# visionml/pytracking

Hardware: AMD Instinct MI355X
Metric: frames/sec DiMP-50 online track (288x288, 5 SD iters) (higher is better)
Workload: dtype f32; 1 GPU; BASELINE configs[1]: DiMP-50 single sequence per GPU; per frame classify(1x512x18x18) + arg-max + memory insert + DiMPSteepestDescentGN(5 it) over n=50x512x18x18, K=4; sequences_per_gpu=1, parallelism=1 independent sequences

## Files before the change

include/pt_hot.h:

```cpp
#ifndef PT_HOT_H
#define PT_HOT_H

#include <stddef.h>
#include <stdint.h>

#ifdef __cplusplus
extern "C" {
#endif

typedef enum pt_status {
    PT_OK = 0,
    PT_ERR_NULL = -1,
    PT_ERR_SHAPE = -2,
    PT_ERR_UNSUPPORTED = -3,
    PT_ERR_WORKSPACE = -4,
    PT_ERR_LAUNCH = -5
} pt_status;

const char* pt_strerror(int status);
int pt_abi_version(void);


size_t pt_apply_filter_ws_bytes(int n, int C, int H, int W, int KH, int KW, int OH, int OW);
int pt_apply_filter_f32(const float* feat, long feat_stride_n, const float* filt, float* scores,
                        int n, int C, int H, int W, int KH, int KW, int OH, int OW,
                        void* ws, size_t ws_bytes, void* stream);

size_t pt_feat_transpose_ws_bytes(int n, int C, int H, int W, int KH, int KW, int OH, int OW);
int pt_feat_transpose_f32(const float* feat, long feat_stride_n, const float* inp, float* grad,
                          int n, int C, int H, int W, int KH, int KW, int OH, int OW,
                          void* ws, size_t ws_bytes, void* stream);


enum { PT_SD_DIMP = 0, PT_SD_DIMP_L2 = 1, PT_SD_PRDIMP = 2 };
enum { PT_ACT_RELU = 0, PT_ACT_BENTPAR = 1 };
enum { PT_MASK_SIGMOID = 0, PT_MASK_LINEAR = 1 };

typedef struct pt_sd_params {
    int   kind;
    float step_length;
    float reg;
    float alpha_eps;
    float feat_stride;
    int   num_bins;
    float bin_displacement;
    const float* label_lut;
    const float* mask_lut;
    const float* spatial_lut;
    int   mask_act;
    int   score_act;
    float act_param;
    float gauss_sigma;
    float hinge_threshold;
    float uni_weight;
    int   normalize_label;
    float label_shrink;
    int   has_softmax_reg;
    float softmax_reg;
    float label_threshold;
} pt_sd_params;

size_t pt_sd_ws_bytes(int n, int C, int H, int W, int K);
int pt_sd_solve_f32(const pt_sd_params* p, const float* w_in, const float* feat, long feat_stride_n,
                    const float* bb, const float* sample_weight,
                    int n, int C, int H, int W, int K, int num_iter,
                    float* w_iters, float* losses, void* ws, size_t ws_bytes, void* stream);

int pt_sd_solve_batch_f32(const pt_sd_params* p, int S, const float* const* w_in, const float* const* feat, long feat_stride_n,
                          const float* const* bb, const float* const* sample_weight, int n, int C, int H, int W, int K,
                          int num_iter, float* const* w_iters, float* const* losses, void* const* ws, size_t ws_bytes_each,
                          void* stream, void* const* aux_streams, int n_aux);

typedef struct {
    int   score_act;
    float act_param;
// ... 226 lines not shown
```

pytracking_amd/_lib.py:

```python
import ctypes
import os
import subprocess

_HERE = os.path.dirname(os.path.abspath(__file__))
LIB_PATH = os.environ.get("PT_HOT_LIB", os.path.join(_HERE, "libpt_hot.so"))
SOURCES = ["filter_kernels.hip", "fast_passes.hip", "sd_solver.hip", "mf_kernels.hip", "lwl_solver.hip", "atom_cg.hip", "atom_gn.hip", "tomp.hip", "localize.hip", "iou_refine.hip", "prroi.hip", "patch.hip", "frame_full.hip", "api.hip", "gn_hinge.hip", "tcm.hip"]
HEADERS = ["common.h", "pt_internal.h", "rbuild.h", "sd_common.h", "mfma_gemm.h", "prroi_dev.h", "localize_dev.h", "frame_mid.h", os.path.join("..", "..", "include", "pt_hot.h")]
HIPCC_FLAGS = ["--offload-arch=gfx950", "-O3", "-std=c++17", "-fPIC", "-Wno-pass-failed", "-mllvm", "-amdgpu-kernarg-preload-count=14"]

PT_SD_DIMP, PT_SD_DIMP_L2, PT_SD_PRDIMP = 0, 1, 2
PT_ERR_NULL, PT_ERR_SHAPE, PT_ERR_UNSUPPORTED, PT_ERR_WORKSPACE, PT_ERR_LAUNCH = -1, -2, -3, -4, -5
PT_ACT_RELU, PT_ACT_BENTPAR = 0, 1
PT_MASK_SIGMOID, PT_MASK_LINEAR = 0, 1

class IouDims(ctypes.Structure):
    _fields_ = [(n, ctypes.c_int) for n in ("C3", "C4", "I3", "I4", "H3", "W3", "H4", "W4")]


class PatchGeom(ctypes.Structure):
    _fields_ = [(n, ctypes.c_int) for n in ("df", "os0", "os1", "tl0", "tl1", "crop_h", "crop_w")]


class AugDesc(ctypes.Structure):
    _fields_ = ([(n, ctypes.c_int) for n in ("kind", "pad_top", "pad_left", "th", "tw", "fs0", "fs1", "tap_off0", "tap_off1",
                                             "reserved")] + [("m", ctypes.c_double * 6)])


PT_AUG_IDENTITY, PT_AUG_FLIP_H, PT_AUG_FLIP_V, PT_AUG_BLUR, PT_AUG_SCALE, PT_AUG_ROTATE = range(6)
PT_AUG_MAX_TAPS = 256


class LocalizeParams(ctypes.Structure):
    _fields_ = ([(n, ctypes.c_double) for n in ("target_not_found_threshold", "uncertain_threshold", "hard_sample_threshold")]
                + [(n, ctypes.c_float) for n in ("distractor_threshold", "hard_negative_threshold", "target_not_found_f32",
                                                 "disp_threshold", "center_r", "center_c", "ratio_r", "ratio_c")]
                + [(n, ctypes.c_float * 8) for n in ("scale", "neigh_r", "neigh_c", "prev_r", "prev_c")])


class LocalizeState(ctypes.Structure):
    _fields_ = ([(n, ctypes.c_double) for n in ("target_not_found_threshold", "uncertain_threshold", "hard_sample_threshold",
                                                "distractor_threshold", "hard_negative_threshold",
                                                "target_neighborhood_scale", "dispalcement_scale")]
                + [(n, ctypes.c_float * 2) for n in ("kernel_size", "img_support_sz", "target_sz", "pos")]
                + [("sample_scales", ctypes.c_float * 8), ("sample_pos", ctypes.c_float * 16)])


PT_LOC_FLAGS = ("normal", "hard_negative", "uncertain", "not_found")


class FrameGlue(ctypes.Structure):
    _fields_ = [("image_sz", ctypes.c_float * 2), ("img_sample_sz", ctypes.c_float * 2), ("target_inside_ratio", ctypes.c_double),
                ("box_jitter_pos", ctypes.c_double), ("box_jitter_sz", ctypes.c_double), ("use_classifier", ctypes.c_int),
                ("num_random", ctypes.c_int), ("rand_u", ctypes.c_float * 60)]


PT_FRAME_HOST_FLOATS = 128


class TompDims(ctypes.Structure):
    _fields_ = [(n, ctypes.c_int) for n in ("d_model", "nhead", "dim_ff", "n_enc", "n_dec", "H", "W", "max_res")]


EXPORTS = [
    "pt_strerror", "pt_abi_version",
    "pt_apply_filter_ws_bytes", "pt_apply_filter_f32",
    "pt_feat_transpose_ws_bytes", "pt_feat_transpose_f32",
    "pt_sd_ws_bytes", "pt_sd_solve_f32",
    "pt_atom_cg_ws_bytes", "pt_atom_cg_f32", "pt_atom_gn_ws_bytes", "pt_atom_gn_f32",
    "pt_prroi_fwd_f32", "pt_prroi_bwd_feat_f32", "pt_prroi_bwd_coor_f32",
    "pt_track_frame_ws_bytes", "pt_track_frame_f32", "pt_track_frame_chain_f32", "pt_track_frame_flush_f32",
    "pt_apply_filter_mf_ws_bytes", "pt_apply_filter_mf_f32", "pt_feat_transpose_mf_ws_bytes", "pt_feat_transpose_mf_f32",
    "pt_lwl_ws_bytes", "pt_lwl_gn_solve_f32",
    "pt_tomp_param_floats", "pt_tomp_prepared_floats", "pt_tomp_prepare_f32", "pt_tomp_posenc_f32", "pt_tomp_predict_ws_bytes", "pt_tomp_predict_f32", "pt_tomp_linear_f32",
    "pt_tomp_bbreg_param_floats", "pt_tomp_bbreg_ws_bytes", "pt_tomp_bbreg_f32",
    "pt_clf_head_ws_bytes", "pt_clf_head_f32", "pt_max2d_f32", "pt_localize_f32", "pt_localize_decide_f32",
    "pt_localize_constants_f32", "pt_localize_advanced_f32", "pt_localize_advanced_sync_f32",
    "pt_iou_param_floats", "pt_iou_prepared_floats", "pt_iou_prepare_f32", "pt_iou_refine_ws_bytes", "pt_iou_refine_f32", "pt_iou_refine_sync_f32",
    "pt_track_frame_replay_pass_f32", "pt_sample_patch_f32", "pt_augment_patches_f32", "pt_track_frame_head_ws_bytes", "pt_track_frame_head_f32",
    "pt_track_frame_full_ws_bytes", "pt_track_frame_full_f32", "pt_track_frame_full_launch_f32", "pt_host_buffer_forget",
    "pt_track_frame_full_dyn_bytes", "pt_track_frame_full_dyn_fill_f32", "pt_host_wait_word_f32",
    "pt_sd_solve_batch_f32", "pt_stream_probe_f32",
    "pt_gn_hinge_ws_bytes", "pt_gn_hinge_solve_f32", "pt_gn_hinge_route",
    "pt_tcm_peaks_f32", "pt_tcm_desc_ws_bytes", "pt_tcm_desc_f32",
    "pt_tcm_match_weight_floats", "pt_tcm_match_ws_bytes", "pt_tcm_match_f32",
]

PT_TCM_MAX_POINTS, PT_TCM_MAX_LAYERS = 64, 32


class TcmMatchParams(ctypes.Structure):
    _fields_ = ([(n, ctypes.c_int) for n in ("M", "N", "n_layers")] + [("layer_types", ctypes.c_uint)]
                + [(n, ctypes.c_int) for n in ("skip_gnn", "sinkhorn_iters")] + [("filter_threshold", ctypes.c_float)]
                + [("kpt_center0", ctypes.c_float * 2), ("kpt_scale0", ctypes.c_float), ("kpt_center1", ctypes.c_float * 2),
                   ("kpt_scale1", ctypes.c_float), ("weight_floats", ctypes.c_size_t)])


class GnHingeParams(ctypes.Structure):
    _fields_ = [("score_act", ctypes.c_int)] + [(n, ctypes.c_float) for n in ("act_param", "hinge_threshold", "activation_leak",
                                                                             "filter_reg", "steplength_reg")]


class FramePending(ctypes.Structure):
    _fields_ = [("iters", ctypes.c_int), ("step_length", ctypes.c_float), ("reg_eps", ctypes.c_float)]


class SdParams(ctypes.Structure):
    _fields_ = [
        ("kind", ctypes.c_int), ("step_length", ctypes.c_float), ("reg", ctypes.c_float),
        ("alpha_eps", ctypes.c_float), ("feat_stride", ctypes.c_float),
        ("num_bins", ctypes.c_int), ("bin_displacement", ctypes.c_float),
        ("label_lut", ctypes.c_void_p), ("mask_lut", ctypes.c_void_p), ("spatial_lut", ctypes.c_void_p),
        ("mask_act", ctypes.c_int), ("score_act", ctypes.c_int), ("act_param", ctypes.c_float),
        ("gauss_sigma", ctypes.c_float), ("hinge_threshold", ctypes.c_float),
        ("uni_weight", ctypes.c_float), ("normalize_label", ctypes.c_int), ("label_shrink", ctypes.c_float),
        ("has_softmax_reg", ctypes.c_int), ("softmax_reg", ctypes.c_float), ("label_threshold", ctypes.c_float),
    ]


# ... 243 lines not shown
```

pytracking_amd/csrc/api.hip:

```cpp
#include <algorithm>
#include <atomic>
#include <chrono>
#include <mutex>
#include <utility>
#include <vector>
#include "common.h"
#include "pt_internal.h"

extern "C" const char* pt_strerror(int status) {
    switch (status) {
        case PT_OK: return "ok";
        case PT_ERR_NULL: return "required pointer is NULL";
        case PT_ERR_SHAPE: return "non-positive or inconsistent dimension";
        case PT_ERR_UNSUPPORTED: return "configuration not covered by the gfx950 kernels";
        case PT_ERR_WORKSPACE: return "workspace too small or not 256-byte aligned";
        case PT_ERR_LAUNCH: return "HIP launch failed";
        default: return "unknown status";
    }
}

extern "C" int pt_abi_version(void) { return 1; }

static std::atomic<const void*> g_pinned_seen[8];
static std::atomic<unsigned> g_pinned_next{0};
// ... 15 lines not shown
    for (auto& s : g_pinned_seen) {
        const void* cur = p;
        s.compare_exchange_strong(cur, nullptr, std::memory_order_acq_rel);
    }
}

bool pt_stream_events(void* main_stream, void* aux_stream, hipEvent_t* fork, hipEvent_t* join) {
    struct Key { int dev; void* main; void* aux; };
    struct Ent { Key k; hipEvent_t fork, join; };
    static std::mutex mu;
    static std::vector<Ent> pool;
    int dev = -1;
    if (hipGetDevice(&dev) != hipSuccess) { (void)hipGetLastError(); return false; }
    std::lock_guard<std::mutex> lk(mu);
    for (auto& e : pool)
        if (e.k.dev == dev && e.k.main == main_stream && e.k.aux == aux_stream) {
            if (fork) *fork = e.fork;
            if (join) *join = e.join;
            return true;
        }
    hipEvent_t a, b;
    if (hipEventCreateWithFlags(&a, hipEventDisableTiming) != hipSuccess) { (void)hipGetLastError(); return false; }
    if (hipEventCreateWithFlags(&b, hipEventDisableTiming) != hipSuccess) {
        (void)hipGetLastError();
        (void)hipEventDestroy(a);
        return false;
    }
    pool.push_back({{dev, main_stream, aux_stream}, a, b});
    if (fork) *fork = a;
    if (join) *join = b;
    return true;
}

int pt_poll_word(volatile float* word, float seq, const void* buf, void* stream) {
    const auto t0 = std::chrono::steady_clock::now();
    for (unsigned spin = 1;; ++spin) {
        if (*word == seq) break;
        __builtin_ia32_pause();
        if ((spin & 0xFFFF) == 0 && std::chrono::steady_clock::now() - t0 > std::chrono::seconds(2)) {
            pt_host_buffer_forget(buf);
            if (hipStreamSynchronize((hipStream_t)stream) != hipSuccess) return PT_ERR_LAUNCH;
            if (*word != seq) return PT_ERR_LAUNCH;
            break;
        }
    }
    __atomic_thread_fence(__ATOMIC_ACQUIRE);
    return PT_OK;
}

static int filt_check(int n, int C, int H, int W, int KH, int KW, int OH, int OW) {
    if (n <= 0 || C <= 0 || H <= 0 || W <= 0 || KH <= 0 || KW <= 0 || OH <= 0 || OW <= 0) return PT_ERR_SHAPE;
    if (OH > H + 2 * (KH / 2) - KH + 1 || OW > W + 2 * (KW / 2) - KW + 1) return PT_ERR_SHAPE;
    if (KH * KW > 16) return PT_ERR_UNSUPPORTED;
    return PT_OK;
}

extern "C" size_t pt_apply_filter_ws_bytes(int n, int C, int H, int W, int KH, int KW, int OH, int OW) {
    if (filt_check(n, C, H, W, KH, KW, OH, OW)) return 0;
    PtPlan p = pt_make_plan(n, C, H, W, KH, KW, OH, OW);
    size_t fl = pt_align_floats(pt_spart_floats(p));
    PtFast f = pt_fast_plan(n, C, H, W, KH, KW, OH, OW);
    if (f.ok) fl = std::max(fl, pt_align_floats(pt_fast_spart_floats(f)));
    return fl * sizeof(float);
}

extern "C" int pt_apply_filter_f32(const float* feat, long feat_stride_n, const float* filt, float* scores, int n, int C,
                                   int H, int W, int KH, int KW, int OH, int OW, void* ws, size_t ws_bytes,
                                   void* stream) {
    if (!feat || !filt || !scores || !ws) return PT_ERR_NULL;
    int rc = filt_check(n, C, H, W, KH, KW, OH, OW);
    if (rc) return rc;
    if (feat_stride_n < (long)C * H * W) return PT_ERR_SHAPE;
    if (ws_bytes < pt_apply_filter_ws_bytes(n, C, H, W, KH, KW, OH, OW) || ((uintptr_t)ws % 256) != 0)
        return PT_ERR_WORKSPACE;
    hipStream_t st = (hipStream_t)stream;
    float* spart = (float*)ws;
    PtFast f = pt_fast_plan(n, C, H, W, KH, KW, OH, OW);
    if (pt_fast_usable(f, feat, feat_stride_n, filt)) {
        rc = pt_launch_corr2(f, feat, feat_stride_n, filt, spart, st);
        if (rc) return rc;
        return pt_launch_sum_slices(spart, scores, f.KSC, (size_t)n * f.OO, st);
    }
    PtPlan p = pt_make_plan(n, C, H, W, KH, KW, OH, OW);
    rc = pt_launch_corr(p, feat, feat_stride_n, filt, spart, st);
    if (rc) return rc;
    return pt_launch_sum_slices(spart, scores, p.KS, (size_t)n * p.OO, st);
}

struct FtCarve { size_t R, gpart, total; };
static FtCarve ft_carve(const PtPlan& p) {
    FtCarve c;
    c.R = 0;
    c.gpart = pt_align_floats(pt_R_floats(p));
    c.total = c.gpart + pt_align_floats(pt_gpart_floats(p));
    return c;
}

extern "C" size_t pt_feat_transpose_ws_bytes(int n, int C, int H, int W, int KH, int KW, int OH, int OW) {
    if (filt_check(n, C, H, W, KH, KW, OH, OW)) return 0;
    PtPlan p = pt_make_plan(n, C, H, W, KH, KW, OH, OW);
    size_t fl = ft_carve(p).total;
    PtFast f = pt_fast_plan(n, C, H, W, KH, KW, OH, OW);
    if (f.ok) fl = std::max(fl, pt_align_floats(pt_fast_gpart_floats(f)));
    return fl * sizeof(float);
}

// ... 215 lines not shown
```

pytracking_amd/csrc/fast_passes.hip:

```cpp
#include "common.h"
#include "pt_internal.h"
#include "sd_common.h"

#ifndef PT_ADJ_WAVES
#define PT_ADJ_WAVES 8
#endif
#ifndef PT_ADJ_UMAX
#define PT_ADJ_UMAX (128 / PT_ADJ_WAVES)
#endif
#ifndef PT_ADJ_UMAX_WIDE
#define PT_ADJ_UMAX_WIDE (192 / PT_ADJ_WAVES)
#endif
#ifndef PT_C2_CD
#define PT_C2_CD 2
#endif
#ifndef PT_C2_MINW
#define PT_C2_MINW 6
#endif
#ifndef PT_ADJ_PD
#define PT_ADJ_PD 3
#endif

#ifdef PT_STAMPS
static unsigned long long* g_pt_stamps = nullptr;
extern "C" void pt_debug_set_stamps(void* p) { g_pt_stamps = (unsigned long long*)p; }
#define PT_STAMP_ARG unsigned long long* stamps;
#define PT_STAMP_SET(a) (a).stamps = g_pt_stamps
#define PT_STAMP(a, k)                                                                                       \
    do {                                                                                                     \
        if ((a).stamps && (threadIdx.x & 63) == 0)                                                           \
            (a).stamps[((long)blockIdx.x * 16 + (threadIdx.x >> 6)) * 8 + (k)] = (unsigned long long)wall_clock64(); \
    } while (0)
#else
#define PT_STAMP_ARG
#define PT_STAMP_SET(a)
#define PT_STAMP(a, k)
#endif
#if defined(PT_STAMPS) && PT_STAMPS == 2
#define PT_STAMP_A(a, k)
#define PT_STAMP_B(a, k) PT_STAMP(a, k)
#else
#define PT_STAMP_A(a, k) PT_STAMP(a, k)
#define PT_STAMP_B(a, k)
#endif

PtFast pt_fast_plan(int n, int C, int H, int W, int KH, int KW, int OH, int OW) {
    PtFast p;
    p.ok = 0;
    p.n = n; p.C = C; p.H = H; p.W = W; p.KH = KH; p.KW = KW; p.OH = OH; p.OW = OW;
    p.HW = H * W; p.KK = KH * KW; p.OO = OH * OW;
    if ((p.HW % 4) != 0 || W < 4 || p.KK > 16) return p;
    if (C != 64 && C != 128 && C != 256 && C != 512 && C != 1024) return p;
    if ((long)n * p.HW >= (1L << 20)) return p;
    if ((long)n * C * p.HW * 4 >= (1L << 31)) return p;
    p.Q = p.HW / 4;
    p.TF = p.Q / 16;
    p.rem = p.Q % 16;
    p.left = (p.rem > 0 && p.rem <= 4) ? 1 : 0;
    p.tiles = p.TF + ((p.rem > 0 && !p.left) ? 1 : 0);
    if (p.TF < 1 || p.tiles > 16) return p;
    p.nh = 2 * p.tiles <= 10 ? 2 : 1;
    p.CX = C / 8;
    p.KSC = 8;
    if (C == 64) { p.CX = C; p.KSC = 1; }
    p.spw = 1;
    if (p.nh == 2 && p.KSC == 8 && p.CX / 4 <= 16 && (n % 2) == 0 && 8 * n > 256) { p.nh = 1; p.spw = 2; }
    p.NK = p.CX / 4 / p.nh;
    if (p.NK > 16) return p;
    p.HWp = 64 * (p.TF + (p.rem > 0 ? 1 : 0)) + 4;
    p.corr_threads = p.spw * p.nh * p.tiles * 64;
    p.corr_lds = ((size_t)p.CX * 16 + (size_t)p.spw * p.nh * p.KK * p.HWp) * sizeof(float);
    p.sa_direct = (KH == 4 && KW == 4 && p.CX * 16 >= 2 * W + 2) ? 1 : 0;
    if (p.sa_direct && p.HWp < p.HW + 2 * W + 2) p.corr_lds += (size_t)(p.HW + 2 * W + 2 - p.HWp) * sizeof(float);
    if (p.corr_lds > 150 * 1024) return p;
    p.CB = C / 16;
    p.bpx = p.CB / 8;
    p.NG = (int)(((long)n * p.HW + 15) / 16);
    p.KSPL = 0;
    p.E = p.OO <= 384 ? 6 : (p.OO <= 576 ? 9 : 16);
    const int umax = p.E == 9 ? PT_ADJ_UMAX_WIDE : PT_ADJ_UMAX;
    for (int ks = 8; ks <= (p.CB < 8 ? 64 : 16); ks *= 2) {
        const int gper = pt_ceil_div(p.NG, ks), U = pt_ceil_div(gper, PT_ADJ_WAVES);
        if (U <= umax) { p.gper = gper; p.U = U; p.KSPL = pt_ceil_div(p.NG, gper); break; }
    }
    if (p.KSPL == 0) return p;
    p.PH = H + KH - 1;
    p.PW = W + KW - 1;
    while ((p.PW % 16) != 8) ++p.PW;
    p.ns_max = (p.gper * 16 + p.HW - 1) / p.HW + 1;
    p.zn = (KH - 1) * p.PW + KW + 4;
    while (((p.ns_max * p.PH * p.PW + p.zn) % 4) != 0) ++p.zn;
    p.adj_lds = ((size_t)p.ns_max * p.PH * p.PW + p.zn + (size_t)5 * 4 * PT_ADJ_WAVES * umax) * sizeof(float);
    if (p.adj_lds > 96 * 1024 || p.OO > 1024) return p;
    if (H > 255 || W > 255 || n > 65535 || p.gper > 65535 || p.PH > 63 || p.PW > 63 || p.zn > 255 || p.ns_max > 63 || KH > 7 || KW > 7)
        return p;
    p.ok = 1;
    return p;
}

__device__ __forceinline__ int fdiv(int v, float inv_d) { return (int)(((float)v + 0.5f) * inv_d); }

struct Corr2Args {
    pt_gcf feat; long stride_n; pt_gcf filt; pt_gf spart;
    int n, C, H, W, KH, KW, OH, OW, CX, TF, rem, tiles, HWp, nh, KSC;
    int sa_direct;
    pt_gcf gpart; int KSPL; pt_gcf w; float reg; float step; pt_gf g_out; pt_gf anum_part;
    int slot; pt_gcf src; pt_gf copy_dst;
    PT_STAMP_ARG
};

__device__ __forceinline__ float corr2_filter_elem(const Corr2Args& a, int KK, int cx0, int e, bool publish, float& gsq) {
    const int cl = e >> 4, tp = e & 15;
    const bool ok = tp < KK;
    const long ge = (long)(cx0 + cl) * KK + (ok ? tp : 0);
    float v;
    if (a.gpart) {
        const long CKK = (long)a.C * KK;
        v = 0.f;
        for (int k = 0; k < a.KSPL; ++k) v += a.gpart[(long)k * CKK + ge];
        v += a.reg * a.w[ge];
        if (ok) {
            gsq += v * v;
            if (publish) a.g_out[ge] = v;
        }
    } else {
        v = a.filt[ge];
    }
    return ok ? v : 0.f;
}

template <int NK, bool LEFT, int FUSE, bool K16, int NH>
__global__ __launch_bounds__(1024, (NK <= 8 && NH == 2 ? PT_C2_MINW : 4)) void k_corr2(const float* h_feat, long h_stride, const float* h_filt, const float* h_w, const float* h_src, int h_slot,
                                                                              unsigned h_dims, unsigned h_geo, unsigned h_aux, Corr2Args a_arg) {
    extern __shared__ __attribute__((aligned(16))) float lds[];
    __shared__ float scratch[16];
    PT_STAMP(a_arg, 0);
    constexpr int EPT = 2;
    constexpr int FP = FUSE > 0 ? FUSE : 1;
    const int hC = (int)(h_dims >> 16), HW = (int)(h_dims & 0xffffu);
    const int h_tiles = (int)(h_geo & 31u), h_TF = (int)((h_geo >> 5) & 31u), h_rem = (int)((h_geo >> 10) & 15u);
    const int h_KSPL = (int)((h_geo >> 14) & 63u);
    const bool ksc16 = ((h_geo >> 20) & 1u) != 0, ksc1 = ((h_geo >> 21) & 1u) != 0, pair = ((h_geo >> 22) & 1u) != 0;
    const int wps = NH * h_tiles;
    const int nthreads = (pair ? 2 : 1) * wps * 64;
    const int hCX = ksc1 ? hC : (ksc16 ? hC >> 4 : hC >> 3), hHWp = 64 * (h_TF + (h_rem > 0 ? 1 : 0)) + 4;
    const int b = blockIdx.x, xc = b & 7, q = b >> 3;
    const int x = ksc1 ? 0 : (ksc16 ? 2 * xc + (q & 1) : xc), i0 = ksc1 ? b : (ksc16 ? q >> 1 : q);
    const int KK = K16 ? 16 : a_arg.KH * a_arg.KW;
    const int lane = threadIdx.x & 63, wave = __builtin_amdgcn_readfirstlane(threadIdx.x >> 6);
    const int kq = lane >> 4, j = lane & 15;
    const int ws = (pair && wave >= wps) ? 1 : 0, wl = wave - ws * wps;
    const int i = pair ? 2 * i0 + ws : i0;
    const int h = wl >= h_tiles ? 1 : 0, t = wl - h * h_tiles;
    const int cx0 = hCX * x;
    const int nsl = hCX * 16;
    float* __restrict__ afilt = lds;
    float* __restrict__ Tl = lds + nsl + (long)(ws * NH + h) * KK * hHWp;
    const bool over = h_src != nullptr && i == h_slot;
    const float* __restrict__ fi = over ? h_src : h_feat + (long)i * h_stride;
    const bool publish = FUSE != 0 && i0 == 0;
    const int h_n = (int)(h_geo >> 23);
    float lz_q = 0.f, lz_an = 0.f;

    constexpr bool k16 = K16;
    const int n4 = nsl >> 1;
    const int e4 = min((int)threadIdx.x, n4 - 1);
    f32x2 part4[FP], wv4 = {0, 0};
    float part[EPT][FP], wv[EPT];
    long gev[EPT];
    bool okv[EPT];
    if (k16) {
        const long g4 = ((long)cx0 * 16 >> 1) + e4;
        if (FUSE > 0) {
            const unsigned ckk_b = (unsigned)hC * 16u * 4u;
            const __amdgpu_buffer_rsrc_t rg = pt_rsrc(h_filt, (unsigned)h_KSPL * ckk_b);
#pragma unroll
            for (int k = 0; k < FP; ++k)
                part4[k] = __builtin_bit_cast(f32x2, __builtin_amdgcn_raw_buffer_load_b64(rg, (unsigned)g4 * 8u, (unsigned)min(k, h_KSPL - 1) * ckk_b, 0));
            wv4 = ((const f32x2*)h_w)[g4];
        } else if (FUSE < 0) {
            part4[0] = ((const f32x2*)h_filt)[g4];
            wv4 = ((const f32x2*)h_w)[g4];
            const float* __restrict__ anp = h_w + h_aux;
            lz_an = lane < (ksc16 ? 16 : (ksc1 ? 1 : 8)) ? anp[lane] : 0.f;
            lz_q = lane < h_n ? anp[64 + lane] : 0.f;
        } else {
            part4[0] = ((const f32x2*)h_filt)[g4];
        }
    } else {
#pragma unroll
        for (int q = 0; q < EPT; ++q) {
            const int e = threadIdx.x + q * nthreads;
            const int ec = min(e, nsl - 1);
            const int cl = ec >> 4, tp = ec & 15;
            okv[q] = e < nsl && tp < KK;
            gev[q] = (long)(cx0 + cl) * KK + (tp < KK ? tp : 0);
            if (FUSE > 0) {
                const long CKK = (long)hC * KK;
#pragma unroll
                for (int k = 0; k < FP; ++k) part[q][k] = h_filt[(long)min(k, h_KSPL - 1) * CKK + gev[q]];
                wv[q] = h_w[gev[q]];
            } else {
                part[q][0] = h_filt[gev[q]];
            }
        }
    }

    constexpr int CD = NK < PT_C2_CD ? NK : PT_C2_CD;
    const int cbase = cx0 + 4 * (h * NK) + kq;
    const int pos = 64 * t + 4 * j;
    const bool pv = pos < HW;
    const __amdgpu_buffer_rsrc_t fr = pt_rsrc(fi, (unsigned)hC * HW * 4u);
    const unsigned fo = ((unsigned)cbase * HW + (pv ? pos : 0)) * 4u;
    const int lpos = 64 * h_TF + j;
    const bool lv = LEFT && t == 0 && j < 4 * h_rem;
    const unsigned lo = lv ? ((unsigned)cbase * HW + lpos) * 4u : 0xFFFFFFF0u - 64u * (unsigned)HW * 4u;
    f32x4 bq[NK];
    float bl[NK];
    auto ldq = [&](int k) {
        bq[k] = pt_bload4(fr, fo + (unsigned)(4 * k) * HW * 4u);
        if (LEFT && t == 0) bl[k] = pt_bload1(fr, lo + (unsigned)(4 * k) * HW * 4u);
    };
    if (LEFT && t == 0) {
#pragma unroll
        for (int k = 0; k < CD; ++k) bl[k] = pt_bload1(fr, lo + (unsigned)(4 * k) * HW * 4u);
    }
#pragma unroll
    for (int k = 0; k < CD; ++k) bq[k] = pt_bload4(fr, fo + (unsigned)(4 * k) * HW * 4u);
    __builtin_amdgcn_sched_barrier(0);
    const Corr2Args a = pt_late_args<Corr2Args>(56);
    PT_STAMP(a, 1);

    float gsq = 0.f;
    if (k16) {
        f32x2 v4;
        if (FUSE > 0) {
            v4 = (f32x2){0, 0};
#pragma unroll
            for (int k = 0; k < FP; ++k)
                if (k < h_KSPL) v4 += part4[k];
            v4 += a.reg * wv4;
            if ((int)threadIdx.x < n4) {
                gsq = v4[0] * v4[0] + v4[1] * v4[1];
                if (publish) ((f32x2*)a.g_out)[((long)cx0 * 16 >> 1) + e4] = v4;
            }
        } else if (FUSE < 0) {
            float qt = 0.f;
            for (int k = lane + 64; k < h_n; k += 64) qt += (h_w + h_aux)[64 + k];
            const float astep = sd_final_astep(lz_q, qt, lz_an, a.step, a.reg);
            v4 = (f32x2){sd_final_apply(part4[0][0], wv4[0], astep), sd_final_apply(part4[0][1], wv4[1], astep)};
            if ((int)threadIdx.x < n4 && publish) ((f32x2*)a.g_out)[((long)cx0 * 16 >> 1) + e4] = v4;
        } else {
            v4 = part4[0];
        }
        if ((int)threadIdx.x < n4) ((f32x2*)afilt)[e4] = v4;
        for (int q4 = threadIdx.x + nthreads; q4 < n4; q4 += nthreads)
            for (int m = 0; m < 2; ++m) afilt[2 * q4 + m] = corr2_filter_elem(a, KK, cx0, 2 * q4 + m, publish, gsq);
    } else {
#pragma unroll
        for (int q = 0; q < EPT; ++q) {
            const int e = threadIdx.x + q * nthreads;
            float v;
            if (FUSE > 0) {
                v = 0.f;
#pragma unroll
                for (int k = 0; k < FP; ++k) v += k < h_KSPL ? part[q][k] : 0.f;
                v += a.reg * wv[q];
                if (okv[q]) {
                    gsq += v * v;
                    if (publish) a.g_out[gev[q]] = v;
                }
            } else {
                v = part[q][0];
            }
            if (e < nsl) afilt[e] = okv[q] ? v : 0.f;
        }
        for (int e = threadIdx.x + EPT * nthreads; e < nsl; e += nthreads)
            afilt[e] = corr2_filter_elem(a, KK, cx0, e, publish, gsq);
    }
    if (FUSE > 0 && publish) {
        const float tot = block_sum(gsq, scratch, nthreads);
        if (threadIdx.x == 0) a.anum_part[x] = tot;
    }
    PT_STAMP(a, 2);
    __syncthreads();
    PT_STAMP(a, 3);

    f32x4 acc0 = {0, 0, 0, 0}, acc1 = {0, 0, 0, 0}, acc2 = {0, 0, 0, 0}, acc3 = {0, 0, 0, 0}, accL = {0, 0, 0, 0};
    float avv[NK];
#pragma unroll
    for (int k = 0; k < NK; ++k) avv[k] = afilt[(4 * (h * NK + k) + kq) * 16 + j];
    __builtin_amdgcn_sched_barrier(0);
#pragma unroll
    for (int k = 0; k < NK; ++k) {
        if (k + CD < NK) ldq(k + CD);
        const float av = avv[k];
        acc0 = mfma16(av, bq[k][0], acc0);
        acc1 = mfma16(av, bq[k][1], acc1);
        acc2 = mfma16(av, bq[k][2], acc2);
        acc3 = mfma16(av, bq[k][3], acc3);
        if (LEFT && t == 0) accL = mfma16(av, bl[k], accL);
    }
    PT_STAMP(a, 4);
    if (over && a.copy_dst) {
        const pt_gf dp = a.copy_dst + pos + (long)cbase * HW;
        if (pv) {
#pragma unroll
            for (int k = 0; k < NK; ++k) *(f32x4*)(dp + (long)(4 * k) * HW) = bq[k];
        }
        if (lv) {
            const pt_gf dl = a.copy_dst + lpos + (long)cbase * HW;
#pragma unroll
            for (int k = 0; k < NK; ++k) dl[(long)(4 * k) * HW] = bl[k];
        }
    }

#pragma unroll
    for (int r = 0; r < 4; ++r) {
        const int row = 4 * kq + r;
        if (row < KK) {
            f32x4 v = {acc0[r], acc1[r], acc2[r], acc3[r]};
            *(f32x4*)(Tl + row * hHWp + pos) = v;
            if (LEFT && t == 0) Tl[row * hHWp + lpos] = accL[r];
        }
    }
    PT_STAMP(a, 5);
    __syncthreads();
    PT_STAMP(a, 6);

    const int ph = a.KH / 2, pw = a.KW / 2, OO = a.OH * a.OW;
    const float inv_ow = 1.0f / (float)a.OW;
    const int nsm = pair ? 2 : 1;
    if (a.KH == 4 && a.KW == 4) {
      for (int s2 = 0; s2 < nsm; ++s2) {
        const float* __restrict__ T0 = lds + nsl + (long)s2 * NH * KK * hHWp;
        const float* __restrict__ T1 = T0 + (long)KK * hHWp;
        const pt_gf out = a.spart + ((long)x * a.n + (pair ? 2 * i0 + s2 : i0)) * OO;
        if (a.sa_direct) {
            const int su = 4 * hHWp + a.W, sv = hHWp + 1;
            for (int o = threadIdx.x; o < OO; o += nthreads) {
                const int y = fdiv(o, inv_ow), xx0 = o - y * a.OW;
                const int base = (y - 2) * a.W + (xx0 - 2);
                float t0[16], t1[16];
#pragma unroll
                for (int u = 0; u < 4; ++u)
#pragma unroll
                    for (int v = 0; v < 4; ++v) {
                        const int idx = base + (u * su + v * sv);
                        t0[u * 4 + v] = T0[idx];
                        if (NH == 2) t1[u * 4 + v] = T1[idx];
                    }
                int rok[4], cok[4];
#pragma unroll
                for (int u = 0; u < 4; ++u) rok[u] = (unsigned)(y + u - 2) < (unsigned)a.H ? -1 : 0;
#pragma unroll
                for (int v = 0; v < 4; ++v) cok[v] = (unsigned)(xx0 + v - 2) < (unsigned)a.W ? -1 : 0;
                __builtin_amdgcn_sched_barrier(0);
                float tv[16];
#pragma unroll
                for (int q = 0; q < 16; ++q) {
                    const float tsum = NH == 2 ? t0[q] + t1[q] : t0[q];
                    tv[q] = __builtin_bit_cast(float, __builtin_bit_cast(int, tsum) & (rok[q >> 2] & cok[q & 3]));
                }
                float s = 0.f;
#pragma unroll
                for (int q = 0; q < 16; ++q) s += tv[q];
                out[o] = s;
            }
            continue;
        }
        for (int o = threadIdx.x; o < OO; o += nthreads) {
            const int y = fdiv(o, inv_ow), xx0 = o - y * a.OW;
            float tv[16];
#pragma unroll
            for (int u = 0; u < 4; ++u) {
                const int yy = y + u - 2;
#pragma unroll
// ... 22 lines not shown
        const int y = fdiv(o, inv_ow), xx0 = o - y * a.OW;
        float s = 0.f;
        for (int u = 0; u < a.KH; ++u) {
            const int yy = y + u - ph;
            if ((unsigned)yy >= (unsigned)a.H) continue;
            for (int v = 0; v < a.KW; ++v) {
                const int xx = xx0 + v - pw;
                if ((unsigned)xx < (unsigned)a.W) {
                    const int idx = (u * a.KW + v) * hHWp + yy * a.W + xx;
                    s += NH == 2 ? T0[idx] + T1[idx] : T0[idx];
                }
            }
        }
        out[o] = s;
      }
    }
}

int pt_launch_corr2(const PtFast& p, const float* feat, long stride_n, const float* filt, float* spart, hipStream_t st,
                    const PtCorrFuse* fuse, int slot, const float* src, float* copy_dst, const PtCorrLazy* lazy) {
    Corr2Args a;
    a.feat = (pt_gcf)feat; a.stride_n = stride_n; a.filt = (pt_gcf)filt; a.spart = (pt_gf)spart;
    a.n = p.n; a.C = p.C; a.H = p.H; a.W = p.W; a.KH = p.KH; a.KW = p.KW; a.OH = p.OH; a.OW = p.OW;
    a.CX = p.CX; a.TF = p.TF; a.rem = p.rem; a.tiles = p.tiles; a.HWp = p.HWp; a.nh = p.nh; a.KSC = p.KSC;
    a.sa_direct = p.sa_direct;
    a.gpart = nullptr; a.KSPL = 0; a.w = nullptr; a.reg = 0.f; a.g_out = nullptr; a.anum_part = nullptr;
    if (fuse) {
        a.gpart = (pt_gcf)fuse->gpart; a.KSPL = fuse->KSPL; a.w = (pt_gcf)fuse->w; a.reg = fuse->reg; a.g_out = (pt_gf)fuse->g_out;
        a.anum_part = (pt_gf)fuse->anum_part;
    }
    a.slot = slot; a.src = (pt_gcf)src; a.copy_dst = (pt_gf)copy_dst;
    a.step = 0.f;
    unsigned h_aux = 0, h_nbits = 0;
    if (lazy) {
        if (fuse || p.KK != 16 || p.n > 511 || p.CX * 8 > p.corr_threads || !lazy->w_prev || !lazy->g || !lazy->anum || !lazy->w_out ||
            lazy->qs != lazy->anum + 64 || lazy->anum < lazy->g || (lazy->anum - lazy->g) > 0x3fffffffL)
            return PT_ERR_UNSUPPORTED;
        if (((uintptr_t)lazy->w_prev % 16) || ((uintptr_t)lazy->g % 16) || ((uintptr_t)lazy->w_out % 16)) return PT_ERR_UNSUPPORTED;
        a.filt = (pt_gcf)lazy->w_prev; a.w = (pt_gcf)lazy->g; a.g_out = (pt_gf)lazy->w_out; a.reg = lazy->reg_eps; a.step = lazy->step;
        h_aux = (unsigned)(lazy->anum - lazy->g);
        h_nbits = (unsigned)p.n << 23;
    }
    PT_STAMP_SET(a);
    if (((uintptr_t)feat % 16) || (stride_n % 4) || ((uintptr_t)src % 16) || ((uintptr_t)copy_dst % 16)) return PT_ERR_UNSUPPORTED;
    if ((long)p.n * stride_n * 4 >= (1L << 31)) return PT_ERR_UNSUPPORTED;
    if (p.KK == 16 && (((uintptr_t)filt % 16) || ((uintptr_t)a.gpart % 16) || ((uintptr_t)a.w % 16) || ((uintptr_t)a.g_out % 16)))
        return PT_ERR_UNSUPPORTED;
    dim3 grid(p.KSC * (p.n / p.spw)), block(p.corr_threads);
    if (p.C >= (1 << 16) || p.HW >= (1 << 16) || p.tiles > 31 || p.TF > 31 || p.rem > 15 || a.KSPL > 16) return PT_ERR_UNSUPPORTED;
    const unsigned h_dims = ((unsigned)p.C << 16) | (unsigned)p.HW;
    const unsigned h_geo = (unsigned)p.tiles | ((unsigned)p.TF << 5) | ((unsigned)p.rem << 10) | ((unsigned)a.KSPL << 14) |
                           ((p.KSC == 16 ? 1u : 0u) << 20) | ((p.KSC == 1 ? 1u : 0u) << 21) | ((p.spw == 2 ? 1u : 0u) << 22) | h_nbits;
#define PT_C2_HOT(FPTR) (const float*)a.feat, a.stride_n, (const float*)(FPTR), (const float*)a.w, (const float*)a.src, a.slot, h_dims, h_geo, h_aux
#define PT_C2G(NKV, LF, KF, NHV)                                                                                    \
    do {                                                                                                         \
        if (lazy) { if constexpr (KF) hipLaunchKernelGGL((k_corr2<NKV, LF, -1, true, NHV>), grid, block, p.corr_lds, st, PT_C2_HOT(a.filt), a); } \
        else if (!a.gpart) hipLaunchKernelGGL((k_corr2<NKV, LF, 0, KF, NHV>), grid, block, p.corr_lds, st, PT_C2_HOT(a.filt), a);             \
        else if (a.KSPL <= 8) hipLaunchKernelGGL((k_corr2<NKV, LF, 8, KF, NHV>), grid, block, p.corr_lds, st, PT_C2_HOT(a.gpart), a);     \
        else hipLaunchKernelGGL((k_corr2<NKV, LF, 16, KF, NHV>), grid, block, p.corr_lds, st, PT_C2_HOT(a.gpart), a);                     \
    } while (0)
#define PT_C2H(NKV, LF, KF)              \
    do {                                 \
        if (p.nh == 2) PT_C2G(NKV, LF, KF, 2); \
        else PT_C2G(NKV, LF, KF, 1);     \
    } while (0)
#define PT_C2F(NKV, LF)                  \
    do {                                 \
        if (p.KK == 16) PT_C2H(NKV, LF, true); \
        else PT_C2H(NKV, LF, false);     \
    } while (0)
#define PT_C2(NKV)                  \
    do {                            \
        if (p.left) PT_C2F(NKV, true); \
        else PT_C2F(NKV, false);    \
    } while (0)
    if (p.NK == 2) PT_C2(2);
    else if (p.NK == 4) PT_C2(4);
    else if (p.NK == 8) PT_C2(8);
    else PT_C2(16);
#undef PT_C2_HOT
#undef PT_C2G
#undef PT_C2H
#undef PT_C2F
#undef PT_C2
    PT_CHECK_LAUNCH();
    return PT_OK;
}

struct Adj2Args {
    const float* feat; long stride_n; float* gpart;
    int n, C, H, W, KH, KW, OH, OW, NG, gper, U, bpx, PH, PW, ns_max, zn;
    const float* inp;
    SdArgs sd;
    int t, want_loss;
    PT_STAMP_ARG
};

struct Adj2SdLate {
    int n, CKK, has_sw, has_softmax_reg;
    float step, reg, alpha_eps, act_param, softmax_reg;
    int pad0;
    pt_gcf sw, s_in, w0;
    pt_gf mask, sws, s, sg, lms, g, lossp, w_iters;
};
struct Adj2Late {
    pt_gf gpart;
    int C, KH, KW, OH, OW, PH, PW, ns_max, zn, t, want_loss, pad1;
    Adj2SdLate sd;
    PT_STAMP_ARG
};
#ifndef PT_STAMPS
static_assert(sizeof(Adj2Late) == 46 * 4, "Adj2Late layout");
#endif

enum { V_PLAIN = 0, V_DIMP_RELU = 1, V_DIMP_BENT = 2, V_L2 = 3, V_PRDIMP = 4 };

template <int E>
struct PReg { f32x4 pk[E]; float s[E], sg[E], sw[E]; };

template <int V, int E>
__device__ __forceinline__ void sdp_load_hot(const float* __restrict__ pkp, int OO, int i, int lane, PReg<E>& r) {
    const long base = (long)i * OO;
#pragma unroll
    for (int e = 0; e < E; ++e) {
        const long q = base + min(lane + 64 * e, OO - 1);
        if (V == V_PLAIN) r.s[e] = pkp[q];
        else r.pk[e] = ((const f32x4*)pkp)[q];
    }
}
template <int V, int E, typename A>
__device__ __forceinline__ void sdp_load_rest(const A& a, int i, int lane, bool home, PReg<E>& r) {
    const int OO = a.OH * a.OW;
    const long base = (long)i * OO;
    const auto sgp = a.t > 0 ? pt_global((const float*)a.sd.sg) : pt_global((const float*)a.sd.s_in);
    if (V == V_DIMP_BENT) {
#pragma unroll
// ... 518 lines not shown
```

pytracking_amd/csrc/pt_internal.h:

```cpp
#pragma once
#include <hip/hip_runtime.h>
#include <stddef.h>
#include <stdint.h>
#include "../../include/pt_hot.h"

struct PtPlan {
    int n, C, H, W, KH, KW, OH, OW;
    int HW, KK, OO;
    int KS, cper;
    int corr_threads;
    size_t corr_lds;
    int NG;
    int KSPL, gper;
    bool vec4;
};

PtPlan pt_make_plan(int n, int C, int H, int W, int KH, int KW, int OH, int OW);

static inline size_t pt_spart_floats(const PtPlan& p) { return (size_t)p.KS * p.n * p.OO; }
static inline size_t pt_R_floats(const PtPlan& p) { return (size_t)p.NG * 256; }
static inline size_t pt_gpart_floats(const PtPlan& p) { return (size_t)p.KSPL * p.C * p.KK; }
static inline size_t pt_align_floats(size_t x) { return (x + 63) & ~(size_t)63; }

struct PtCorrFuse {
    const float* gpart;
    int KSPL;
    const float* w;
    float reg;
    float* g_out;
    float* anum_part;
    float* copy_dst;
    const float* feat2;
    const float* filt2;
    float* spart2;
};

struct PtInputGrad { const float* v; const float* filt; float* out; int n, Kc, H, W, K; };

int pt_launch_corr(const PtPlan& p, const float* feat, long stride_n, const float* filt, float* spart, hipStream_t st,
                   const PtCorrFuse* fuse = nullptr);
int pt_launch_adj(const PtPlan& p, const float* feat, long stride_n, const float* R, float* gpart, hipStream_t st,
                  const PtInputGrad* ig = nullptr);
int pt_launch_sum_slices(const float* part, float* out, int slices, size_t count, hipStream_t st);
int pt_launch_build_R(const PtPlan& p, const float* inp, float* R, hipStream_t st);

struct PtFast {
    int ok;
    int n, C, H, W, KH, KW, OH, OW, HW, KK, OO, Q;
    int CX, NK, TF, rem, tiles, left, HWp, corr_threads, nh;
    int spw;
    int sa_direct;
    int KSC;
    size_t corr_lds;
    int CB, bpx, NG, KSPL, gper, U, PH, PW, ns_max, E, zn;
    size_t adj_lds;
};
PtFast pt_fast_plan(int n, int C, int H, int W, int KH, int KW, int OH, int OW);
static inline bool pt_fast_usable(const PtFast& f, const void* feat, long stride_n, const void* filt = nullptr,
                                  const void* src = nullptr) {
    return f.ok && ((uintptr_t)feat % 16) == 0 && (stride_n % 4) == 0 && (long)f.n * stride_n * 4 < (1L << 31) &&
           ((uintptr_t)src % 16) == 0 && (f.KK != 16 || ((uintptr_t)filt % 16) == 0);
}
static inline bool pt_sd_route_fast(const PtFast& f, const void* feat, long stride_n, const void* w_in, const void* w_iters,
                                    const void* src, bool label_map) {
    return pt_fast_usable(f, feat, stride_n, w_in, src) && ((uintptr_t)w_iters % 16) == 0 && f.KSPL <= 16 && (!label_map || f.OO <= 1024);
}
static inline size_t pt_fast_spart_floats(const PtFast& p) { return (size_t)16 * p.n * p.OO; }
static inline size_t pt_fast_gpart_floats(const PtFast& p) { return (size_t)p.KSPL * p.C * p.KK; }
struct PtCorrLazy { const float* w_prev; const float* g; const float* anum; const float* qs; float step, reg_eps; float* w_out; };
int pt_launch_corr2(const PtFast& p, const float* feat, long stride_n, const float* filt, float* spart, hipStream_t st,
                    const PtCorrFuse* fuse = nullptr, int slot = -1, const float* src = nullptr,
                    float* copy_dst = nullptr, const PtCorrLazy* lazy = nullptr);
int pt_launch_adj2_plain(const PtFast& p, const float* feat, long stride_n, const float* inp, float* gpart,
                         hipStream_t st);
struct SdArgs;
int pt_launch_adj2_sd(const PtFast& p, const float* feat, long stride_n, const SdArgs& sd, int t, int want_loss,
                      hipStream_t st, bool fuse_init = false);
bool pt_adj2_init_fusable(const PtFast& p, const SdArgs& sd);

size_t pt_mf_gpart_floats(int n, int F, int C, int H, int W, int K);
int pt_mf_groups(int n, int F, int C, int H, int W, int K);
size_t pt_mf_wt_floats(int C, int K);
__host__ __device__ inline long pt_mf_wt_index(int c, int f, int tap, int KK) {
    return ((long)(c >> 2) * 64 + (c & 3) * 16 + f) * (KK == 1 ? 1 : 12) + tap;
}
int pt_launch_mf_wtrans(const float* filt, float* wT, int F, int C, int K, hipStream_t st, int groups = 1,
                        float* clear2 = nullptr);
int pt_mf_corr_tm_splits(int n, int Ftot, int C, int H, int W);
int pt_mf_corr_tm_cost(int n, int Ftot, int C, int H, int W);
int pt_launch_mf_corr_tm(const float* feat, long stride_n, const float* w_tap_major, float* part, int n, int Ftot, int C,
                         int H, int W, int ksplit, hipStream_t st);
int pt_launch_mf_corr1_direct(const float* feat, long stride_n, const float* filt, float* scores, int n, int Ftot, int C,
                              int H, int W, hipStream_t st, long out_stride_n);
int pt_mf_corr_splits(int n, int F, int C, int H, int W, int K);
size_t pt_mf_corr_part_floats(int n, int F, int C, int H, int W, int K);
#define PT_MF_SQ_PARTS 256
struct PtMfSq { const float* sw; int sw_mode; float sw_scalar; long per_image; float* out; int* done; };
int pt_launch_mf_corr(const float* feat, long stride_n, const float* wT, float* scores, int n, int F, int C, int H,
                      int W, int K, hipStream_t st, long out_stride_n = 0, int groups = 1, float* part = nullptr,
                      const PtMfSq* sq = nullptr);
int pt_launch_mf_adj(const float* feat, long stride_n, const float* inp, float* gpart, int n, int F, int C, int H, int W,
                     int K, hipStream_t st, long inp_stride_n = 0, int groups = 1);

// ... 74 lines not shown
```

Before: 9538 frames/s.

## Add mixed half-width wave mapping to corr2 kernel for paired-sample five-tile plans

Introduces a MIX variant of the correlation kernel used when spw==2, tiles==5, KK==16. The first four waves each handle a two-column half of tile 0 (b64 loads, half the MFMAs) and the remaining waves cover the other tiles across the two samples, giving 12 waves instead of 10. The aim is to rebalance per-wave work so the tile carrying the left remainder does not set the critical path. It also adds a plan-query export and widens the debug stamp record with a hardware register read.

Measured after the change: 9672 frames/s (median of 6 runs). +1.4%, better.

```diff
diff --git a/include/pt_hot.h b/include/pt_hot.h
--- a/include/pt_hot.h
+++ b/include/pt_hot.h
@@ -21,6 +21,7 @@
 int pt_abi_version(void);
 
 
+int pt_corr_pass_plan(int n, int C, int H, int W, int KH, int KW, int OH, int OW, int* out);
 size_t pt_apply_filter_ws_bytes(int n, int C, int H, int W, int KH, int KW, int OH, int OW);
 int pt_apply_filter_f32(const float* feat, long feat_stride_n, const float* filt, float* scores,
                         int n, int C, int H, int W, int KH, int KW, int OH, int OW,
diff --git a/pytracking_amd/_lib.py b/pytracking_amd/_lib.py
--- a/pytracking_amd/_lib.py
+++ b/pytracking_amd/_lib.py
@@ -63,7 +63,7 @@
 
 EXPORTS = [
     "pt_strerror", "pt_abi_version",
-    "pt_apply_filter_ws_bytes", "pt_apply_filter_f32",
+    "pt_corr_pass_plan", "pt_apply_filter_ws_bytes", "pt_apply_filter_f32",
     "pt_feat_transpose_ws_bytes", "pt_feat_transpose_f32",
     "pt_sd_ws_bytes", "pt_sd_solve_f32",
     "pt_atom_cg_ws_bytes", "pt_atom_cg_f32", "pt_atom_gn_ws_bytes", "pt_atom_gn_f32",
diff --git a/pytracking_amd/csrc/api.hip b/pytracking_amd/csrc/api.hip
--- a/pytracking_amd/csrc/api.hip
+++ b/pytracking_amd/csrc/api.hip
@@ -91,6 +91,15 @@
     if (n <= 0 || C <= 0 || H <= 0 || W <= 0 || KH <= 0 || KW <= 0 || OH <= 0 || OW <= 0) return PT_ERR_SHAPE;
     if (OH > H + 2 * (KH / 2) - KH + 1 || OW > W + 2 * (KW / 2) - KW + 1) return PT_ERR_SHAPE;
     if (KH * KW > 16) return PT_ERR_UNSUPPORTED;
+    return PT_OK;
+}
+
+extern "C" int pt_corr_pass_plan(int n, int C, int H, int W, int KH, int KW, int OH, int OW, int* out) {
+    if (!out) return PT_ERR_NULL;
+    const PtFast f = pt_fast_plan(n, C, H, W, KH, KW, OH, OW);
+    const int v[10] = {f.ok, f.ok ? f.tiles : 0, f.ok ? f.nh : 0, f.ok ? f.spw : 0, f.ok ? f.mix : 0, f.ok ? f.corr_threads : 0,
+                       f.ok ? f.NK : 0, f.ok ? f.KSC : 0, f.ok ? (int)f.corr_lds : 0, f.ok ? f.left : 0};
+    for (int k = 0; k < 10; ++k) out[k] = v[k];
     return PT_OK;
 }
 
diff --git a/pytracking_amd/csrc/fast_passes.hip b/pytracking_amd/csrc/fast_passes.hip
--- a/pytracking_amd/csrc/fast_passes.hip
+++ b/pytracking_amd/csrc/fast_passes.hip
@@ -1,6 +1,7 @@
 #include "common.h"
 #include "pt_internal.h"
 #include "sd_common.h"
+#include <type_traits>
 
 #ifndef PT_ADJ_WAVES
 #define PT_ADJ_WAVES 8
@@ -28,8 +29,11 @@
 #define PT_STAMP_SET(a) (a).stamps = g_pt_stamps
 #define PT_STAMP(a, k)                                                                                       \
     do {                                                                                                     \
-        if ((a).stamps && (threadIdx.x & 63) == 0)                                                           \
-            (a).stamps[((long)blockIdx.x * 16 + (threadIdx.x >> 6)) * 8 + (k)] = (unsigned long long)wall_clock64(); \
+        if ((a).stamps && (threadIdx.x & 63) == 0) {                                                         \
+            unsigned long long* sp_ = (a).stamps + ((long)blockIdx.x * 16 + (threadIdx.x >> 6)) * 16;        \
+            sp_[(k)] = (unsigned long long)wall_clock64();                                                   \
+            if ((k) == 0) sp_[8] = (unsigned long long)__builtin_amdgcn_s_getreg((31 << 11) | 4) | (1ull << 32); \
+        }                                                                                                    \
     } while (0)
 #else
 #define PT_STAMP_ARG
@@ -67,8 +71,9 @@
     if (p.nh == 2 && p.KSC == 8 && p.CX / 4 <= 16 && (n % 2) == 0 && 8 * n > 256) { p.nh = 1; p.spw = 2; }
     p.NK = p.CX / 4 / p.nh;
     if (p.NK > 16) return p;
+    p.mix = (p.spw == 2 && p.tiles == 5 && p.KK == 16 && p.NK >= 4) ? 1 : 0;
     p.HWp = 64 * (p.TF + (p.rem > 0 ? 1 : 0)) + 4;
-    p.corr_threads = p.spw * p.nh * p.tiles * 64;
+    p.corr_threads = p.mix ? (2 * p.tiles + 2) * 64 : p.spw * p.nh * p.tiles * 64;
     p.corr_lds = ((size_t)p.CX * 16 + (size_t)p.spw * p.nh * p.KK * p.HWp) * sizeof(float);
     p.sa_direct = (KH == 4 && KW == 4 && p.CX * 16 >= 2 * W + 2) ? 1 : 0;
     if (p.sa_direct && p.HWp < p.HW + 2 * W + 2) p.corr_lds += (size_t)(p.HW + 2 * W + 2 - p.HWp) * sizeof(float);
@@ -129,7 +134,7 @@
     return ok ? v : 0.f;
 }
 
-template <int NK, bool LEFT, int FUSE, bool K16, int NH>
+template <int NK, bool LEFT, int FUSE, bool K16, int NH, bool MIX = false>
 __global__ __launch_bounds__(1024, (NK <= 8 && NH == 2 ? PT_C2_MINW : 4)) void k_corr2(const float* h_feat, long h_stride, const float* h_filt, const float* h_w, const float* h_src, int h_slot,
                                                                               unsigned h_dims, unsigned h_geo, unsigned h_aux, Corr2Args a_arg) {
     extern __shared__ __attribute__((aligned(16))) float lds[];
@@ -142,20 +147,24 @@
     const int h_KSPL = (int)((h_geo >> 14) & 63u);
     const bool ksc16 = ((h_geo >> 20) & 1u) != 0, ksc1 = ((h_geo >> 21) & 1u) != 0, pair = ((h_geo >> 22) & 1u) != 0;
     const int wps = NH * h_tiles;
-    const int nthreads = (pair ? 2 : 1) * wps * 64;
+    const int nthreads = MIX ? (2 * h_tiles + 2) * 64 : (pair ? 2 : 1) * wps * 64;
     const int hCX = ksc1 ? hC : (ksc16 ? hC >> 4 : hC >> 3), hHWp = 64 * (h_TF + (h_rem > 0 ? 1 : 0)) + 4;
     const int b = blockIdx.x, xc = b & 7, q = b >> 3;
     const int x = ksc1 ? 0 : (ksc16 ? 2 * xc + (q & 1) : xc), i0 = ksc1 ? b : (ksc16 ? q >> 1 : q);
     const int KK = K16 ? 16 : a_arg.KH * a_arg.KW;
     const int lane = threadIdx.x & 63, wave = __builtin_amdgcn_readfirstlane(threadIdx.x >> 6);
     const int kq = lane >> 4, j = lane & 15;
-    const int ws = (pair && wave >= wps) ? 1 : 0, wl = wave - ws * wps;
+    const bool half = MIX && wave < 4;
+    const int ws = MIX ? (half ? wave >> 1 : (wave - 4 >= h_tiles - 1 ? 1 : 0)) : ((pair && wave >= wps) ? 1 : 0);
+    const int wl = wave - ws * wps;
     const int i = pair ? 2 * i0 + ws : i0;
-    const int h = wl >= h_tiles ? 1 : 0, t = wl - h * h_tiles;
+    const int h = MIX ? (half ? wave & 1 : 0) : (wl >= h_tiles ? 1 : 0);
+    const int t = MIX ? (half ? 0 : wave - 3 - ws * (h_tiles - 1)) : wl - h * h_tiles;
+    const bool lt = LEFT && t == 0 && (!MIX || h == 0);
     const int cx0 = hCX * x;
     const int nsl = hCX * 16;
     float* __restrict__ afilt = lds;
-    float* __restrict__ Tl = lds + nsl + (long)(ws * NH + h) * KK * hHWp;
+    float* __restrict__ Tl = lds + nsl + (long)(ws * NH + (MIX ? 0 : h)) * KK * hHWp;
     const bool over = h_src != nullptr && i == h_slot;
     const float* __restrict__ fi = over ? h_src : h_feat + (long)i * h_stride;
     const bool publish = FUSE != 0 && i0 == 0;
@@ -207,26 +216,34 @@
     }
 
     constexpr int CD = NK < PT_C2_CD ? NK : PT_C2_CD;
-    const int cbase = cx0 + 4 * (h * NK) + kq;
-    const int pos = 64 * t + 4 * j;
+    const int cbase = cx0 + 4 * ((MIX ? 0 : h) * NK) + kq;
+    const int pos = 64 * t + 4 * j + (half ? 2 * h : 0);
     const bool pv = pos < HW;
     const __amdgpu_buffer_rsrc_t fr = pt_rsrc(fi, (unsigned)hC * HW * 4u);
     const unsigned fo = ((unsigned)cbase * HW + (pv ? pos : 0)) * 4u;
     const int lpos = 64 * h_TF + j;
-    const bool lv = LEFT && t == 0 && j < 4 * h_rem;
+    const bool lv = lt && j < 4 * h_rem;
     const unsigned lo = lv ? ((unsigned)cbase * HW + lpos) * 4u : 0xFFFFFFF0u - 64u * (unsigned)HW * 4u;
     f32x4 bq[NK];
     float bl[NK];
+    auto ldf = [&](int k) {
+        if (MIX && half) {
+            const f32x2 v = __builtin_bit_cast(f32x2, __builtin_amdgcn_raw_buffer_load_b64(fr, fo + (unsigned)(4 * k) * HW * 4u, 0, 0));
+            bq[k] = (f32x4){v[0], v[1], 0.f, 0.f};
+        } else {
+            bq[k] = pt_bload4(fr, fo + (unsigned)(4 * k) * HW * 4u);
+        }
+    };
     auto ldq = [&](int k) {
-        bq[k] = pt_bload4(fr, fo + (unsigned)(4 * k) * HW * 4u);
-        if (LEFT && t == 0) bl[k] = pt_bload1(fr, lo + (unsigned)(4 * k) * HW * 4u);
+        ldf(k);
+        if (lt) bl[k] = pt_bload1(fr, lo + (unsigned)(4 * k) * HW * 4u);
     };
-    if (LEFT && t == 0) {
+    if (lt) {
 #pragma unroll
         for (int k = 0; k < CD; ++k) bl[k] = pt_bload1(fr, lo + (unsigned)(4 * k) * HW * 4u);
     }
 #pragma unroll
-    for (int k = 0; k < CD; ++k) bq[k] = pt_bload4(fr, fo + (unsigned)(4 * k) * HW * 4u);
+    for (int k = 0; k < CD; ++k) ldf(k);
     __builtin_amdgcn_sched_barrier(0);
     const Corr2Args a = pt_late_args<Corr2Args>(56);
     PT_STAMP(a, 1);
@@ -286,43 +303,61 @@
     __syncthreads();
     PT_STAMP(a, 3);
 
-    f32x4 acc0 = {0, 0, 0, 0}, acc1 = {0, 0, 0, 0}, acc2 = {0, 0, 0, 0}, acc3 = {0, 0, 0, 0}, accL = {0, 0, 0, 0};
-    float avv[NK];
-#pragma unroll
-    for (int k = 0; k < NK; ++k) avv[k] = afilt[(4 * (h * NK + k) + kq) * 16 + j];
-    __builtin_amdgcn_sched_barrier(0);
-#pragma unroll
-    for (int k = 0; k < NK; ++k) {
-        if (k + CD < NK) ldq(k + CD);
-        const float av = avv[k];
-        acc0 = mfma16(av, bq[k][0], acc0);
-        acc1 = mfma16(av, bq[k][1], acc1);
-        acc2 = mfma16(av, bq[k][2], acc2);
-        acc3 = mfma16(av, bq[k][3], acc3);
-        if (LEFT && t == 0) accL = mfma16(av, bl[k], accL);
-    }
-    PT_STAMP(a, 4);
-    if (over && a.copy_dst) {
-        const pt_gf dp = a.copy_dst + pos + (long)cbase * HW;
-        if (pv) {
-#pragma unroll
-            for (int k = 0; k < NK; ++k) *(f32x4*)(dp + (long)(4 * k) * HW) = bq[k];
-        }
-        if (lv) {
-            const pt_gf dl = a.copy_dst + lpos + (long)cbase * HW;
-#pragma unroll
-            for (int k = 0; k < NK; ++k) dl[(long)(4 * k) * HW] = bl[k];
-        }
-    }
-
-#pragma unroll
-    for (int r = 0; r < 4; ++r) {
-        const int row = 4 * kq + r;
-        if (row < KK) {
-            f32x4 v = {acc0[r], acc1[r], acc2[r], acc3[r]};
-            *(f32x4*)(Tl + row * hHWp + pos) = v;
-            if (LEFT && t == 0) Tl[row * hHWp + lpos] = accL[r];
-        }
+    auto mfma_phase = [&](auto half_c) {
+        constexpr bool HALF = decltype(half_c)::value;
+        f32x4 acc0 = {0, 0, 0, 0}, acc1 = {0, 0, 0, 0}, acc2 = {0, 0, 0, 0}, acc3 = {0, 0, 0, 0}, accL = {0, 0, 0, 0};
+        float avv[NK];
+#pragma unroll
+        for (int k = 0; k < NK; ++k) avv[k] = afilt[(4 * ((MIX ? 0 : h) * NK + k) + kq) * 16 + j];
+        __builtin_amdgcn_sched_barrier(0);
+#pragma unroll
+        for (int k = 0; k < NK; ++k) {
+            if (k + CD < NK) ldq(k + CD);
+            const float av = avv[k];
+            acc0 = mfma16(av, bq[k][0], acc0);
+            acc1 = mfma16(av, bq[k][1], acc1);
+            if constexpr (!HALF) {
+                acc2 = mfma16(av, bq[k][2], acc2);
+                acc3 = mfma16(av, bq[k][3], acc3);
+            }
+            if (lt) accL = mfma16(av, bl[k], accL);
+        }
+        PT_STAMP(a, 4);
+        if (over && a.copy_dst) {
+            const pt_gf dp = a.copy_dst + pos + (long)cbase * HW;
+            if (pv) {
+#pragma unroll
+                for (int k = 0; k < NK; ++k) {
+                    if constexpr (HALF) *(f32x2*)(dp + (long)(4 * k) * HW) = (f32x2){bq[k][0], bq[k][1]};
+                    else *(f32x4*)(dp + (long)(4 * k) * HW) = bq[k];
+                }
+            }
+            if (lv) {
+                const pt_gf dl = a.copy_dst + lpos + (long)cbase * HW;
+#pragma unroll
+                for (int k = 0; k < NK; ++k) dl[(long)(4 * k) * HW] = bl[k];
+            }
+        }
+
+#pragma unroll
+        for (int r = 0; r < 4; ++r) {
+            const int row = 4 * kq + r;
+            if (row < KK) {
+                if constexpr (HALF) {
+                    *(f32x2*)(Tl + row * hHWp + pos) = (f32x2){acc0[r], acc1[r]};
+                } else {
+                    f32x4 v = {acc0[r], acc1[r], acc2[r], acc3[r]};
+                    *(f32x4*)(Tl + row * hHWp + pos) = v;
+                }
+                if (lt) Tl[row * hHWp + lpos] = accL[r];
+            }
+        }
+    };
+    if constexpr (MIX) {
+        if (half) mfma_phase(std::true_type{});
+        else mfma_phase(std::false_type{});
+    } else {
+        mfma_phase(std::false_type{});
     }
     PT_STAMP(a, 5);
     __syncthreads();
@@ -451,17 +486,17 @@
     const unsigned h_geo = (unsigned)p.tiles | ((unsigned)p.TF << 5) | ((unsigned)p.rem << 10) | ((unsigned)a.KSPL << 14) |
                            ((p.KSC == 16 ? 1u : 0u) << 20) | ((p.KSC == 1 ? 1u : 0u) << 21) | ((p.spw == 2 ? 1u : 0u) << 22) | h_nbits;
 #define PT_C2_HOT(FPTR) (const float*)a.feat, a.stride_n, (const float*)(FPTR), (const float*)a.w, (const float*)a.src, a.slot, h_dims, h_geo, h_aux
-#define PT_C2G(NKV, LF, KF, NHV)                                                                                    \
+#define PT_C2G(NKV, LF, KF, NHV, MX)                                                                                  \
     do {                                                                                                         \
-        if (lazy) { if constexpr (KF) hipLaunchKernelGGL((k_corr2<NKV, LF, -1, true, NHV>), grid, block, p.corr_lds, st, PT_C2_HOT(a.filt), a); } \
-        else if (!a.gpart) hipLaunchKernelGGL((k_corr2<NKV, LF, 0, KF, NHV>), grid, block, p.corr_lds, st, PT_C2_HOT(a.filt), a);             \
-        else if (a.KSPL <= 8) hipLaunchKernelGGL((k_corr2<NKV, LF, 8, KF, NHV>), grid, block, p.corr_lds, st, PT_C2_HOT(a.gpart), a);     \
-        else hipLaunchKernelGGL((k_corr2<NKV, LF, 16, KF, NHV>), grid, block, p.corr_lds, st, PT_C2_HOT(a.gpart), a);                     \
+        if (lazy) { if constexpr (KF) hipLaunchKernelGGL((k_corr2<NKV, LF, -1, true, NHV, MX>), grid, block, p.corr_lds, st, PT_C2_HOT(a.filt), a); } \
+        else if (!a.gpart) hipLaunchKernelGGL((k_corr2<NKV, LF, 0, KF, NHV, MX>), grid, block, p.corr_lds, st, PT_C2_HOT(a.filt), a);             \
+        else if (a.KSPL <= 8) hipLaunchKernelGGL((k_corr2<NKV, LF, 8, KF, NHV, MX>), grid, block, p.corr_lds, st, PT_C2_HOT(a.gpart), a);     \
+        else hipLaunchKernelGGL((k_corr2<NKV, LF, 16, KF, NHV, MX>), grid, block, p.corr_lds, st, PT_C2_HOT(a.gpart), a);                     \
     } while (0)
 #define PT_C2H(NKV, LF, KF)              \
     do {                                 \
-        if (p.nh == 2) PT_C2G(NKV, LF, KF, 2); \
-        else PT_C2G(NKV, LF, KF, 1);     \
+        if (p.nh == 2) PT_C2G(NKV, LF, KF, 2, false); \
+        else PT_C2G(NKV, LF, KF, 1, false);     \
     } while (0)
 #define PT_C2F(NKV, LF)                  \
     do {                                 \
@@ -473,7 +508,17 @@
         if (p.left) PT_C2F(NKV, true); \
         else PT_C2F(NKV, false);    \
     } while (0)
-    if (p.NK == 2) PT_C2(2);
+#define PT_C2M(NKV)                                  \
+    do {                                             \
+        if (p.left) PT_C2G(NKV, true, true, 1, true);   \
+        else PT_C2G(NKV, false, true, 1, true);      \
+    } while (0)
+    if (p.mix) {
+        if (p.NK == 4) PT_C2M(4);
+        else if (p.NK == 8) PT_C2M(8);
+        else PT_C2M(16);
+    }
+    else if (p.NK == 2) PT_C2(2);
     else if (p.NK == 4) PT_C2(4);
     else if (p.NK == 8) PT_C2(8);
     else PT_C2(16);
@@ -481,6 +526,7 @@
 #undef PT_C2G
 #undef PT_C2H
 #undef PT_C2F
+#undef PT_C2M
 #undef PT_C2
     PT_CHECK_LAUNCH();
     return PT_OK;
diff --git a/pytracking_amd/csrc/pt_internal.h b/pytracking_amd/csrc/pt_internal.h
--- a/pytracking_amd/csrc/pt_internal.h
+++ b/pytracking_amd/csrc/pt_internal.h
@@ -49,6 +49,7 @@
     int n, C, H, W, KH, KW, OH, OW, HW, KK, OO, Q;
     int CX, NK, TF, rem, tiles, left, HWp, corr_threads, nh;
     int spw;
+    int mix;
     int sa_direct;
     int KSC;
     size_t corr_lds;
```
